# SchusterLab/qoc

Hardware: AMD Instinct MI355X
Metric: propagator-steps/sec (fwd+grad), dim=32 Schroedinger, 1000 steps x 256 seeds (higher is better)
Workload: dtype f64

## Files before the change

### qoc_amd/csrc/qocx_action.hip

```cpp
#include "qocx_action_core.h"

namespace qocx {

namespace action {

#define QOCX_SCALAR_MEM __attribute__((address_space(4)))
typedef const QOCX_SCALAR_MEM int* ScalarInts;
typedef const QOCX_SCALAR_MEM double* ScalarDoubles;

static __device__ __forceinline__ double inv_p(int p) {
    constexpr InvTable table;
    return table.v[p];
}

__device__ __forceinline__ void dpp_cmac16(double& r0, double& i0, double& r1, double& i1, double xr, double xi,
                                           const double (&ar)[16], const double (&ai)[16]) {
#define QOCX_ACTION_CMAC(R, I, C)                                                                          \
    "v_fmac_f64_dpp %[" R "], %[xr], %[ar" #C "] row_newbcast:" #C " row_mask:0xf bank_mask:0xf\n\t"         \
    "v_fmac_f64_dpp %[" I "], %[xi], %[ar" #C "] row_newbcast:" #C " row_mask:0xf bank_mask:0xf\n\t"         \
    "v_fmac_f64_dpp %[" R "], -%[xi], %[ai" #C "] row_newbcast:" #C " row_mask:0xf bank_mask:0xf\n\t"        \
    "v_fmac_f64_dpp %[" I "], %[xr], %[ai" #C "] row_newbcast:" #C " row_mask:0xf bank_mask:0xf\n\t"
#define QOCX_ACTION_CMAC2(C, D) QOCX_ACTION_CMAC("r0", "i0", C) QOCX_ACTION_CMAC("r1", "i1", D)
#define QOCX_ACTION_COL(C) [ar##C] "v"(ar[C]), [ai##C] "v"(ai[C])
    asm("s_nop 1\n\t" QOCX_ACTION_CMAC2(0, 1) QOCX_ACTION_CMAC2(2, 3) QOCX_ACTION_CMAC2(4, 5) QOCX_ACTION_CMAC2(6, 7)
            QOCX_ACTION_CMAC2(8, 9) QOCX_ACTION_CMAC2(10, 11) QOCX_ACTION_CMAC2(12, 13) QOCX_ACTION_CMAC2(14, 15)
        : [r0] "+v"(r0), [i0] "+v"(i0), [r1] "+v"(r1), [i1] "+v"(i1)
        : [xr] "v"(xr), [xi] "v"(xi), QOCX_ACTION_COL(0), QOCX_ACTION_COL(1), QOCX_ACTION_COL(2), QOCX_ACTION_COL(3),
          QOCX_ACTION_COL(4), QOCX_ACTION_COL(5), QOCX_ACTION_COL(6), QOCX_ACTION_COL(7), QOCX_ACTION_COL(8),
          QOCX_ACTION_COL(9), QOCX_ACTION_COL(10), QOCX_ACTION_COL(11), QOCX_ACTION_COL(12), QOCX_ACTION_COL(13),
          QOCX_ACTION_COL(14), QOCX_ACTION_COL(15));
#undef QOCX_ACTION_COL
#undef QOCX_ACTION_CMAC2
#undef QOCX_ACTION_CMAC
}

template <int NB, int KR, bool EXACT>
static __device__ __forceinline__ void action_sweep_body(const ActionArgs& args, double2* turn) {
    typedef Geo<NB> G;
    constexpr int NP = G::NP, CPL = G::CPL, H = G::H;
    const SweepArgs& sw = args.sw;
    const int b = blockIdx.x;
    const int lane = lane_id(), i = lane % NP, h = lane / NP;
    const bool g0 = (h == 0);
    const int nsteps = sw.nsteps, K = EXACT ? KR : args.K, m_max = args.m_max;
    const int jb = sw.j_begin, je = sw.j_end;
    const double dt = args.dt;
    __builtin_amdgcn_s_setprio(3);

    static_assert(NB == 2 && CPL == 16, "one block of 16 columns per lane group");
    auto image_at = [&](int cc) { return ((16 * h + cc) / H) * 64 + ((16 * h + cc) % H) * NP + i; };
    double h0r[CPL], h0i[CPL], gr[KR][CPL], gi[KR][CPL];
#pragma unroll
    for (int cc = 0; cc < CPL; ++cc) {
        const double2 e = args.h0_rimg[image_at(cc)];
        h0r[cc] = dt * e.y;
        h0i[cc] = -dt * e.x;
    }
#pragma unroll
    for (int k = 0; k < KR; ++k)
#pragma unroll
        for (int cc = 0; cc < CPL; ++cc) {
            const double2 e = k < K ? args.g_rimg[(size_t)k * G::MAT + image_at(cc)] : make_double2(0, 0);
            gr[k][cc] = dt * e.y;
            gi[k][cc] = -dt * e.x;
        }

    const ScalarInts words = (ScalarInts)(sw.s_arr + (size_t)b * nsteps);
    const ScalarDoubles u_b = (ScalarDoubles)(args.ustep + (size_t)b * nsteps * K);
    struct StepHead {
        int word;
        double u[KR];
    };
    auto fetch = [&](int step) __attribute__((always_inline)) {
        StepHead s;
        s.word = words[step];
#pragma unroll
        for (int k = 0; k < KR; ++k) s.u[k] = k < K ? u_b[(size_t)step * K + k] : 0.0;
        return s;
    };
    double are[CPL], aim[CPL];
    auto build = [&](int step, const StepHead& s) __attribute__((always_inline)) {
        if constexpr (EXACT) {
#pragma unroll
            for (int cc = 0; cc < CPL; ++cc) {
                double r = h0r[cc], im = h0i[cc];
#pragma unroll
                for (int k = 0; k < KR; ++k) {
                    r = fma(s.u[k], gr[k][cc], r);
                    im = fma(s.u[k], gi[k][cc], im);
                }
                are[cc] = r;
                aim[cc] = im;
            }
        } else {
#pragma unroll
            for (int cc = 0; cc < CPL; ++cc) {
                are[cc] = h0r[cc];
                aim[cc] = h0i[cc];
            }
#pragma unroll
            for (int k = 0; k < KR; ++k)
                if (k < K) {
                    const double uk = s.u[k];
#pragma unroll
                    for (int cc = 0; cc < CPL; ++cc) {
                        are[cc] = fma(uk, gr[k][cc], are[cc]);
                        aim[cc] = fma(uk, gi[k][cc], aim[cc]);
                    }
                }
            for (int k = KR; k < K; ++k) {
                const double uk = u_b[(size_t)step * K + k] * dt;
#pragma unroll
                for (int cc = 0; cc < CPL; ++cc) {
                    const double2 e = args.g_rimg[(size_t)k * G::MAT + image_at(cc)];
                    are[cc] = fma(uk, e.y, are[cc]);
                    aim[cc] = fma(-uk, e.x, aim[cc]);
                }
            }
        }
    };
    auto matvec = [&](double xr, double xi, double& yr, double& yi) __attribute__((always_inline)) {
        const double sxr = spread_halves(xr, h), sxi = spread_halves(xi, h);
        double s0r = 0, s0i = 0, s1r = 0, s1i = 0;
        dpp_cmac16(s0r, s0i, s1r, s1i, sxr, sxi, are, aim);
        yr = sum_groups<NB>(s0r + s1r);
        yi = sum_groups<NB>(s0i + s1i);
    };
    double vr = 0, vi = 0;
    int count = 0;
    auto step_apply = [&](int step, const StepHead& s, double sign, double2* keep_base)
                          __attribute__((always_inline)) {
        const int m = step_degree(__builtin_amdgcn_readfirstlane(s.word));
        if (m < 1 || m > m_max) return false;
        build(step, s);
        double2* keep = keep_base ? keep_base + ((size_t)b * nsteps + step) * m_max * NP : nullptr;
        count += (lane == m) ? 1 : 0;
        double sr = vr, si = vi;
        for (int p = 1; p <= m; ++p) {
            const double f = sign * inv_p(p);
            if (keep != nullptr && g0) keep[(size_t)(p - 1) * NP + i] = make_double2(vr, vi);
            double yr, yi;
            matvec(vr, vi, yr, yi);
            vr = f * yr;
            vi = f * yi;
            sr += vr;
            si += vi;
        }
        vr = sr;
        vi = si;
        return true;
    };
    auto refuse = [&]() {
        if (lane == 0) atomicOr(sw.status, 8);
    };

    if (sw.phase & 1) {
        const double2 p0 = jb == 0 ? sw.psi0[i] : args.carry_f[(size_t)b * NP + i];
        vr = p0.x;
        vi = p0.y;
        StepHead head = fetch(jb);
        for (int step = jb; step < je; ++step) {
            const StepHead next = fetch(step + 1 < je ? step + 1 : step);
            if (!step_apply(step, head, 1.0, args.kv_f)) {
                refuse();
                return;
            }
            head = next;
        }
        if (count > 0 && lane <= MMAX) atomicAdd(args.degree_counts + lane, count);
        if (je == nsteps) {
            turn[i] = make_double2(vr, vi);
            wave_sync();
            const double cost = eval_costs<NB>(sw, false, true, turn, nullptr, h, i);
            if (sw.unit_adjoint && sw.want_grad) unit_adjoint_scales<NB>(sw, turn, b, h, i);
            if (g0) sw.final_out[(size_t)b * NP + i] = make_double2(vr, vi);
            if (lane == 0) sw.cost_out[b] = cost;
        } else if (g0) {
            args.carry_f[(size_t)b * NP + i] = make_double2(vr, vi);
        }
    }
    if (!(sw.phase & 2)) return;

    wave_sync();
    if (je == nsteps) {
        unit_adjoint_seed<NB>(sw, turn, 0, 1, h, i);
        wave_sync();
        const double2 t = turn[i];
        vr = t.x;
        vi = t.y;
    } else {
        const double2 t = sw.lam_buf[(size_t)b * NP + i];
        vr = t.x;
        vi = t.y;
    }
    StepHead head = fetch(je - 1);
    for (int step = je - 1; step >= jb; --step) {
        const StepHead next = fetch(step - 1 >= jb ? step - 1 : step);
        if (!step_apply(step, head, -1.0, args.kv_b)) {
            refuse();
            return;
        }
        head = next;
    }
    if (jb > 0 && g0) sw.lam_buf[(size_t)b * NP + i] = make_double2(vr, vi);
}

template <int NB, int KR>
__global__ __launch_bounds__(64) void action_sweep_kernel(ActionArgs args) {
    __shared__ __attribute__((aligned(16))) double2 turn[Geo<NB>::NP];
    action_sweep_body<NB, KR, false>(args, turn);
}

template <int NB>
__global__ __launch_bounds__(64) void action_sweep_exact_kernel(ActionArgs args) {
    __shared__ __attribute__((aligned(16))) double2 turn[Geo<NB>::NP];
    action_sweep_body<NB, 2, true>(args, turn);
}

template <int NB>
__global__ __launch_bounds__(64) __attribute__((amdgpu_waves_per_eu(5, 5))) void action_grad_kernel(
    ActionGradArgs args) {
    typedef Geo<NB> G;
    constexpr int NP = G::NP, CPL = G::CPL, H = G::H, GB = 4;
    static_assert(H == 2, "the two lane groups share the terms of rho");
    extern __shared__ __attribute__((aligned(16))) char smem[];
    double2* vl = reinterpret_cast<double2*>(smem);
    double2* rho = vl + (size_t)args.m_max * NP;
    const int step = args.step0 + blockIdx.x, b = blockIdx.y;
    const int lane = lane_id(), i = lane % NP, h = lane / NP;
    const int K = args.K;
    const size_t idx = (size_t)b * args.nsteps + step;
    const int m = step_degree(args.s_arr[idx]);
    if (m < 1 || m > args.m_max) return;
    const double2* vf = args.kv_f + idx * args.m_max * NP;
    const double2* wb = args.kv_b + idx * args.m_max * NP;
    double2 tv = wb[i];
    for (int l0 = h; l0 < m + h; l0 += 4 * H) {
        double2 t[4];
#pragma unroll
        for (int q = 0; q < 4; ++q) t[q] = vf[(size_t)min(l0 + q * H, m - 1) * NP + i];
        asm volatile("" : "+v"(t[0].x), "+v"(t[0].y), "+v"(t[1].x), "+v"(t[1].y), "+v"(t[2].x), "+v"(t[2].y),
                          "+v"(t[3].x), "+v"(t[3].y));
#pragma unroll
        for (int q = 0; q < 4; ++q)
            if (l0 + q * H < m) vl[(l0 + q * H) * NP + i] = t[q];
    }
    double abr[CPL], abi[CPL];
#pragma unroll
    for (int cc = 0; cc < CPL; ++cc) {
        abr[cc] = 0;
        abi[cc] = 0;
    }
    wave_sync();
    for (int ii = 0; ii < m; ++ii) {
        double rr = 0, ri = 0;
        for (int l0 = 0; l0 < m - ii; l0 += H) {
            const double c0 = COEF.c[ii * MMAX + l0], c1 = COEF.c[ii * MMAX + l0 + 1];
            const double c = h == 0 ? c0 : c1;
            const int l = l0 + h;
            if (l < m - ii) {
                const double2 v = vl[l * NP + i];
                rr = fma(c, v.x, rr);
                ri = fma(c, v.y, ri);
            }
        }
        rr = sum_groups<NB>(rr);
        ri = sum_groups<NB>(ri);
        double2* slot = rho + (ii & 1) * NP;
        slot[i] = make_double2(rr, ri);
        wave_sync();
        const double2 w = tv;
        if (ii + 1 < m) tv = wb[(size_t)(ii + 1) * NP + i];
#pragma unroll
        for (int c0 = 0; c0 < CPL; c0 += GB) {
            double2 r[GB];
#pragma unroll
            for (int cc = 0; cc < GB; ++cc) r[cc] = slot[(c0 + cc) * H + h];
#pragma unroll
            for (int cc = 0; cc < GB; ++cc) {
                abr[c0 + cc] = fma(w.y, r[cc].y, fma(w.x, r[cc].x, abr[c0 + cc]));
                abi[c0 + cc] = fma(-w.x, r[cc].y, fma(w.y, r[cc].x, abi[c0 + cc]));
            }
        }
    }
    const double dts = args.dt;
    for (int k = 0; k < K; ++k) {
        double acc = 0, acc_im = 0;
#pragma unroll
        for (int c0 = 0; c0 < CPL; c0 += GB) {
            double2 e[GB];
#pragma unroll
            for (int cc = 0; cc < GB; ++cc) e[cc] = args.g_rimg[(size_t)k * G::MAT + (c0 + cc) * 64 + lane];
            asm volatile("" ::: "memory");
#pragma unroll
            for (int cc = 0; cc < GB; ++cc) {
                acc = fma(abi[c0 + cc], -dts * e[cc].x, fma(abr[c0 + cc], dts * e[cc].y, acc));
                acc_im = fma(abi[c0 + cc], -dts * e[cc].y, fma(abr[c0 + cc], -dts * e[cc].x, acc_im));
            }
        }
        acc = wave_sum(acc);
        acc_im = wave_sum(acc_im);
        if (lane == 0) {
            args.gstep[(idx * K + k) * 2] = acc;
            args.gstep[(idx * K + k) * 2 + 1] = acc_im;
        }
    }
}

}

int action_grad_lds_bytes(int m_max) { return (m_max + 2) * Geo<2>::NP * (int)sizeof(double2); }

void launch_action_sweep(const ActionArgs& a, int batch, hipStream_t st) {
    if (batch <= 0 || a.sw.j_end <= a.sw.j_begin) return;
    if (a.K == 2)
        hipLaunchKernelGGL((action::action_sweep_exact_kernel<2>), dim3(batch), dim3(64), 0, st, a);
    else
        hipLaunchKernelGGL((action::action_sweep_kernel<2, 2>), dim3(batch), dim3(64), 0, st, a);
}

void launch_action_grad(const ActionGradArgs& a, int nsteps, int batch, hipStream_t st) {
    if (batch <= 0 || nsteps <= 0) return;
    hipLaunchKernelGGL((action::action_grad_kernel<2>), dim3(nsteps, batch), dim3(64),
                       action_grad_lds_bytes(a.m_max), st, a);
}

}
```

### qoc_amd/csrc/qocx_action_core.h

```cpp
#ifndef QOCX_ACTION_CORE_H
#define QOCX_ACTION_CORE_H

#include "qocx_sweep_common.h"
#include "qocx_action.h"

namespace qocx {

namespace action {

constexpr int MMAX = QOCX_ACTION_MAX_DEGREE;

struct InvTable {
    double v[MMAX + 2];
    constexpr InvTable() : v{} {
        for (int p = 1; p < MMAX + 2; ++p) v[p] = 1.0 / (double)p;
    }
};
struct CoefTable {
    double c[MMAX * MMAX];
    constexpr CoefTable() : c{} {
        for (int i = 0; i < MMAX; ++i) {
            double v = 1.0 / (double)(i + 1);
            c[i * MMAX] = v;
            for (int l = 1; l < MMAX; ++l) {
                v = v * (double)l / (double)(i + l + 1);
                c[i * MMAX + l] = v;
            }
        }
    }
};
__device__ __constant__ const InvTable INV_P = InvTable();
__device__ __constant__ const CoefTable COEF = CoefTable();

template <int K0>
__device__ __forceinline__ void dpp_cmac4(double& r0, double& i0, double& r1, double& i1, double xr, double xi,
                                          double a0r, double a0i, double a1r, double a1i, double a2r,
                                          double a2i, double a3r, double a3i) {
#define QOCX_ACTION_CMAC(R, I, AR, AI, BC)                                                        \
    "v_fmac_f64_dpp %[" R "], %[xr], %[" AR "] row_newbcast:%[" BC "] row_mask:0xf bank_mask:0xf\n\t"  \
    "v_fmac_f64_dpp %[" I "], %[xi], %[" AR "] row_newbcast:%[" BC "] row_mask:0xf bank_mask:0xf\n\t"  \
    "v_fmac_f64_dpp %[" R "], -%[xi], %[" AI "] row_newbcast:%[" BC "] row_mask:0xf bank_mask:0xf\n\t" \
    "v_fmac_f64_dpp %[" I "], %[xr], %[" AI "] row_newbcast:%[" BC "] row_mask:0xf bank_mask:0xf\n\t"
    asm("s_nop 1\n\t" QOCX_ACTION_CMAC("r0", "i0", "a0r", "a0i", "k0") QOCX_ACTION_CMAC("r1", "i1", "a1r", "a1i", "k1")
            QOCX_ACTION_CMAC("r0", "i0", "a2r", "a2i", "k2") QOCX_ACTION_CMAC("r1", "i1", "a3r", "a3i", "k3")
        : [r0] "+v"(r0), [i0] "+v"(i0), [r1] "+v"(r1), [i1] "+v"(i1)
        : [xr] "v"(xr), [xi] "v"(xi), [a0r] "v"(a0r), [a0i] "v"(a0i), [a1r] "v"(a1r), [a1i] "v"(a1i),
          [a2r] "v"(a2r), [a2i] "v"(a2i), [a3r] "v"(a3r), [a3i] "v"(a3i), [k0] "i"(K0), [k1] "i"(K0 + 1),
          [k2] "i"(K0 + 2), [k3] "i"(K0 + 3));
#undef QOCX_ACTION_CMAC
}

__device__ __forceinline__ double spread_halves(double v, int h) {
    const unsigned lo = (unsigned)__double2loint(v), hi = (unsigned)__double2hiint(v);
    auto a = __builtin_amdgcn_permlane16_swap(lo, lo, false, false);
    auto b = __builtin_amdgcn_permlane16_swap(hi, hi, false, false);
    return h == 0 ? make_f64((int)a[0], (int)b[0]) : make_f64((int)a[1], (int)b[1]);
}

}

}

#endif
```

### qoc_amd/csrc/qocx_api.hip

```cpp
#include <dlfcn.h>
#include <unistd.h>

#include <cfloat>

#include "qocx_host.h"
#include "qocx_action.h"

namespace {

thread_local std::string g_error;

}

namespace qocx::host {

int fail(int code, const std::string& msg) {
    g_error = msg;
    return code;
}

const double THETA13 = 5.371920351148152;

int pade_scale_count(double norm1) {
    int s = 0;
// ... 1180 lines not shown
    }
    std::vector<double2> padded((size_t)batch * count * S * np, make_double2(0, 0));
    for (size_t v = 0; v < (size_t)batch * count * S; ++v)
        for (int i = 0; i < n; ++i)
            padded[v * np + i] = make_double2(bars[2 * (v * n + i)], bars[2 * (v * n + i) + 1]);
    if (ctx->inj_index.upload(index, ctx->stream) || ctx->inj_bars.upload(padded, ctx->stream))
        return QOCX_ERR_HIP;
    ctx->inj_count = count;
    ctx->inj_batch = batch;
    return 0;
}

int qocx_set_chunk(qocx_ctx* ctx, int32_t seeds_per_chunk) {
    if (!ctx) return fail(QOCX_ERR_ARG, "ctx is NULL");
    ctx->chunk_user = seeds_per_chunk < 0 ? 0 : seeds_per_chunk;
    return 0;
}

int qocx_set_pipeline(qocx_ctx* ctx, int32_t time_segments) {
    if (!ctx) return fail(QOCX_ERR_ARG, "ctx is NULL");
    ctx->pipe_user = time_segments < 0 ? 0 : time_segments;
    return 0;
}

int qocx_set_keep_step_states(qocx_ctx* ctx, int32_t keep) {
    if (!ctx) return fail(QOCX_ERR_ARG, "ctx is NULL");
    ctx->keep_step_states = keep ? 1 : 0;
    return 0;
}

static int eval_seeds(qocx_ctx* ctx, int32_t want_grad) {
    if (ctx->seeds.M == 0) return eval_items(ctx, want_grad);
    if (!ctx->has_problem || ctx->B < 1) return fail(QOCX_ERR_STATE, "no problem / controls");
    HIP_TRY(hipSetDevice(ctx->device));
    const int seeds = ctx->ens_B;
    if (ctx->ens_stale)
        if (int rc = ensemble_expand(ctx, seeds)) return rc;
    if (int rc = eval_items(ctx, want_grad)) return rc;
    if (ctx->ens_cost.ensure((size_t)seeds) ||
        (ctx->have_grads && ctx->ens_grads.ensure((size_t)seeds * ctx->nc * ctx->seeds.Kr)))
        return QOCX_ERR_HIP;
    SeedBuffers buf = seed_buffers(ctx);
    if (!ctx->have_grads) buf.grads = nullptr;
    if (ctx->seeds.sweep()) qocx::launch_sweep_reduce(sweep_args(ctx->seeds, ctx->nc, buf), ctx->stream);
    else qocx::launch_ensemble_reduce(ensemble_args(ctx->seeds, seeds, ctx->nc, buf), ctx->stream);
    HIP_TRY(hipGetLastError());
    HIP_TRY(hipStreamSynchronize(ctx->stream));
    return 0;
}

int qocx_eval_resident(qocx_ctx* ctx, int32_t want_grad) {
    if (!ctx) return fail(QOCX_ERR_ARG, "ctx is NULL");
    if (int rc = eval_seeds(ctx, want_grad)) return rc;
    ControlCosts& cc = ctx->control_costs;
    if (cc.count == 0) return duration_finish(ctx);
    const int seeds = seed_count(ctx);
    if (int rc = run_control_costs(ctx, cc, seeds, ctx->nc, seed_channels(ctx), seed_controls(ctx), ctx->have_grads))
        return rc;
    qocx::launch_add_control_costs(seed_costs(ctx), cc.cost.p, ctx->have_grads ? seed_grads(ctx) : nullptr,
                                   cc.grad.p, seeds, (size_t)ctx->nc * seed_channels(ctx), ctx->stream);
    HIP_TRY(hipGetLastError());
    HIP_TRY(hipStreamSynchronize(ctx->stream));
    return duration_finish(ctx);
}

int qocx_download_results(qocx_ctx* ctx, double* cost_out, double* grad_out, double* final_out) {
    if (!ctx) return fail(QOCX_ERR_ARG, "ctx is NULL");
    if (!ctx->have_results) return fail(QOCX_ERR_STATE, "no evaluation results");
    HIP_TRY(hipSetDevice(ctx->device));
    const int B = ctx->B, np = ctx->np, S = ctx->S, n = ctx->n, seeds = seed_count(ctx);
    if (cost_out)
        HIP_TRY(hipMemcpyAsync(cost_out, seed_costs(ctx), (size_t)seeds * sizeof(double),
                               hipMemcpyDeviceToHost, ctx->stream));
    if (grad_out) {
        if (!ctx->have_grads) return fail(QOCX_ERR_STATE, "gradients were not computed");
        HIP_TRY(hipMemcpyAsync(grad_out, seed_grads(ctx),
                               (size_t)seeds * ctx->nc * seed_channels(ctx) * sizeof(double),
                               hipMemcpyDeviceToHost, ctx->stream));
    }
    std::vector<double2> fin;
    if (final_out) {
        fin.resize((size_t)B * S * np);
        HIP_TRY(hipMemcpyAsync(fin.data(), ctx->final_out.p, fin.size() * sizeof(double2),
                               hipMemcpyDeviceToHost, ctx->stream));
    }
    HIP_TRY(hipStreamSynchronize(ctx->stream));
    if (final_out)
        for (size_t v = 0; v < (size_t)B * S; ++v)
            for (int i = 0; i < n; ++i) {
                final_out[2 * (v * n + i)] = fin[v * np + i].x;
                final_out[2 * (v * n + i) + 1] = fin[v * np + i].y;
            }
    return 0;
}

int qocx_download_step_states(qocx_ctx* ctx, double* states_out) {
    if (!ctx || !states_out) return fail(QOCX_ERR_ARG, "NULL argument");
    if (!ctx->have_results || !ctx->have_step_states)
        return fail(QOCX_ERR_STATE, "step states were not kept (qocx_set_keep_step_states)");
    HIP_TRY(hipSetDevice(ctx->device));
    const size_t nvec = (size_t)ctx->B * (ctx->nsteps + 1) * ctx->S;
    std::vector<double2> tmp(nvec * ctx->np);
    HIP_TRY(hipMemcpy(tmp.data(), ctx->step_states.p, tmp.size() * sizeof(double2),
                      hipMemcpyDeviceToHost));
    for (size_t v = 0; v < nvec; ++v)
        for (int i = 0; i < ctx->n; ++i) {
            states_out[2 * (v * ctx->n + i)] = tmp[v * ctx->np + i].x;
            states_out[2 * (v * ctx->n + i) + 1] = tmp[v * ctx->np + i].y;
        }
    return 0;
}

int qocx_eval_schroedinger(qocx_ctx* ctx, int32_t batch, const double* controls, int32_t want_grad,
                           double* cost_out, double* grad_out, double* final_out) {
    int rc = qocx_upload_controls(ctx, batch, controls);
    if (rc) return rc;
    rc = eval_seeds(ctx, want_grad);
    if (rc) return rc;
    if ((rc = duration_finish(ctx))) return rc;
    return qocx_download_results(ctx, cost_out, (want_grad && ctx->K > 0) ? grad_out : nullptr,
                                 final_out);
}

int qocx_set_timing(qocx_ctx* ctx, int32_t enable) {
    if (!ctx) return fail(QOCX_ERR_ARG, "ctx is NULL");
    if (enable < 0 || enable > 8) return fail(QOCX_ERR_ARG, "timing mode must be 0, 1 or 2 + kernel index");
    ctx->timing = enable;
    ctx->time_active = false;
    return 0;
}

int qocx_get_timing(qocx_ctx* ctx, int32_t which, int64_t* launches, double* total_ms) {
    if (!ctx || which < 0 || which > 6) return fail(QOCX_ERR_ARG, "bad argument");
    if (launches) *launches = ctx->t_launch[which];
    if (total_ms) *total_ms = ctx->t_ms[which];
    return 0;
}

int qocx_reset_timing(qocx_ctx* ctx) {
    if (!ctx) return fail(QOCX_ERR_ARG, "ctx is NULL");
    for (int i = 0; i < 7; ++i) {
        ctx->t_launch[i] = 0;
        ctx->t_ms[i] = 0;
    }
    return 0;
}

static const char* const kVariantKnobs[] = {
    "sweep_impl", "sweep_one", "sweep_dense", "sweep_inverse", "sweep_inverse_small", "sweep_umode", "bidir",
    "unit_adjoint", "latency", "fuse_lu", "lu_inverse", "lu_mfma", "lu_dpp", "pack8", "m4_linear", "magnus_4w",
    "pade_order", "k1a_three", "k1a_four", "k1a_share", "k1a_herm4", "general_split", "general_skew",
    "lindblad_two_sided", "lindblad_side_limit", "lindblad_q2", "lindblad_chain", "lindblad_real_ops", "lindblad_4t",
    "lindblad_hermitian", "lindblad_pad_operator", "action", "action_states", "action_costs",
    "action_degree"};
static const char* const kDiagKnobs[] = {"dbg_skip", "sweep3_dbg", "sweep3_stamps", "lindblad_stamps",
                                         "k1a_stamps", "k1a_dbg", "peak_mode"};

int qocx_knob_kind(const char* name) {
    if (!name) return 0;
    for (const char* k : kVariantKnobs)
        if (strcmp(k, name) == 0) return 1;
    for (const char* k : kDiagKnobs)
        if (strcmp(k, name) == 0) return qocx::kDiagBuild ? 2 : -2;
    return 0;
}

int qocx_build_is_diag(void) { return qocx::kDiagBuild ? 1 : 0; }

int qocx_debug_set_knob(qocx_ctx* ctx, const char* name, int64_t value) {
    if (!ctx || !name) return fail(QOCX_ERR_ARG, "NULL argument");
    const int kind = qocx_knob_kind(name);
    if (kind > 0) {
        if (strcmp(name, "action_states") == 0 && value != 0 && (value < 2 || value > QOCX_ACTION_MAX_STATES))
            return fail(QOCX_ERR_ARG, "action_states must be 0 or 2 .. 4 (QOCX_ACTION_MAX_STATES)");
        if (strcmp(name, "action_costs") == 0 && value != 0 && value != 1)
            return fail(QOCX_ERR_ARG, "action_costs must be 0 or 1");
        if (strcmp(name, "action_degree") == 0 && value != 0 && value != 1)
            return fail(QOCX_ERR_ARG, "action_degree must be 0 or 1");
        ctx->knobs[name] = value;
        return 0;
    }
    if (kind == -2)
        return fail(QOCX_ERR_ARG, std::string("diagnostic knob '") + name +
                                      "' exists in libqocx_diag.so only (make diag, -DQOCX_DIAG)");
    return fail(QOCX_ERR_ARG, std::string("unknown knob: ") + name);
}


int qocx_comm_unique_id(uint8_t* id128) {
    if (!id128) return fail(QOCX_ERR_ARG, "id128 is NULL");
    qocx_ctx tmp;
    int rc = load_rccl(&tmp);
    if (rc) return rc;
    int e = tmp.rccl.GetUniqueId((void*)id128);
    if (e != 0) return fail(QOCX_ERR_RCCL, "ncclGetUniqueId failed");
    return 0;
}

int qocx_comm_init(qocx_ctx* ctx, const uint8_t* id128, int32_t rank, int32_t world) {
    if (!ctx || !id128) return fail(QOCX_ERR_ARG, "NULL argument");
    HIP_TRY(hipSetDevice(ctx->device));
    int rc = load_rccl(ctx);
    if (rc) return rc;
    typedef int (*init_fn)(void**, int, ncclUniqueIdBytes, int);
    init_fn f = (init_fn)dlsym(ctx->rccl.lib, "ncclCommInitRank");
    ncclUniqueIdBytes uid;
    memcpy(uid.internal, id128, 128);
    if (world < 1 || rank < 0 || rank >= world) return fail(QOCX_ERR_ARG, "rank / world out of range");
    if (!f) return fail(QOCX_ERR_RCCL, "librccl has no ncclCommInitRank");
    if (getenv("QOCX_RCCL_DEBUG")) {
        unsigned long long sum = 1469598103934665603ull;
        for (int i = 0; i < 128; ++i) sum = (sum ^ id128[i]) * 1099511628211ull;
        char bus[64] = "?";
        (void)hipDeviceGetPCIBusId(bus, sizeof(bus), ctx->device);
        int version = 0;
        typedef int (*ver_fn)(int*);
        if (ver_fn v = (ver_fn)dlsym(ctx->rccl.lib, "ncclGetVersion")) (void)v(&version);
        const char* ipc = getenv("HSA_ENABLE_IPC_MODE_LEGACY");
        fprintf(stderr, "[qocx rccl] ncclCommInitRank rank=%d world=%d hip_device=%d pci=%s id_fnv=%016llx "
                        "rccl_version=%d HSA_ENABLE_IPC_MODE_LEGACY=%s pid=%d\n",
                rank, world, ctx->device, bus, sum, version, ipc ? ipc : "(unset)", (int)getpid());
        fflush(stderr);
    }
    int e = f(&ctx->comm, world, uid, rank);
    if (e != 0)
        return fail(QOCX_ERR_RCCL, std::string("ncclCommInitRank: ") +
                                       (ctx->rccl.GetErrorString ? ctx->rccl.GetErrorString(e) : "?"));
    return 0;
}

static int comm_allreduce(qocx_ctx* ctx, double* buf, int64_t count, int op) {
    if (!ctx || !buf || count < 1) return fail(QOCX_ERR_ARG, "bad argument");
    if (!ctx->comm) return fail(QOCX_ERR_STATE, "communicator not initialised");
    HIP_TRY(hipSetDevice(ctx->device));
    if (ctx->comm_buf.ensure((size_t)count)) return QOCX_ERR_HIP;
    HIP_TRY(hipMemcpyAsync(ctx->comm_buf.p, buf, count * sizeof(double), hipMemcpyHostToDevice,
                           ctx->stream));
    int e = ctx->rccl.AllReduce(ctx->comm_buf.p, ctx->comm_buf.p, (size_t)count, 8, op, ctx->comm,
                                ctx->stream);
    if (e != 0)
        return fail(QOCX_ERR_RCCL, std::string("ncclAllReduce: ") +
                                       (ctx->rccl.GetErrorString ? ctx->rccl.GetErrorString(e) : "?"));
    HIP_TRY(hipMemcpyAsync(buf, ctx->comm_buf.p, count * sizeof(double), hipMemcpyDeviceToHost,
                           ctx->stream));
    HIP_TRY(hipStreamSynchronize(ctx->stream));
    return 0;
}

int qocx_download_costs(qocx_ctx* ctx, double* cost_out) {
    if (!ctx || !cost_out) return fail(QOCX_ERR_ARG, "NULL argument");
    if (!ctx->have_results) return fail(QOCX_ERR_STATE, "no evaluation results");
    HIP_TRY(hipSetDevice(ctx->device));
    HIP_TRY(hipMemcpyAsync(cost_out, seed_costs(ctx), (size_t)seed_count(ctx) * sizeof(double),
                           hipMemcpyDeviceToHost, ctx->stream));
    HIP_TRY(hipStreamSynchronize(ctx->stream));
    return 0;
}

int qocx_ensemble_download_members(qocx_ctx* ctx, double* cost_out) {
    if (!ctx || !cost_out) return fail(QOCX_ERR_ARG, "NULL argument");
    if (ctx->seeds.M == 0 || ctx->seeds.swp_B > 0) return fail(QOCX_ERR_STATE, "no ensemble set (qocx_set_ensemble)");
    if (!ctx->have_results) return fail(QOCX_ERR_STATE, "no evaluation results");
    HIP_TRY(hipSetDevice(ctx->device));
    HIP_TRY(hipMemcpyAsync(cost_out, ctx->cost_out.p, (size_t)ctx->B * sizeof(double),
                           hipMemcpyDeviceToHost, ctx->stream));
    HIP_TRY(hipStreamSynchronize(ctx->stream));
    return 0;
}

int qocx_sweep_download_sensitivities(qocx_ctx* ctx, double* scales_out, double* offsets_out) {
    if (!ctx) return fail(QOCX_ERR_ARG, "ctx is NULL");
    if (ctx->seeds.swp_B == 0) return fail(QOCX_ERR_STATE, "no sweep set (qocx_set_sweep)");
    if (!ctx->have_results || !ctx->have_grads || ctx->ens_stale)
        return fail(QOCX_ERR_STATE, "sweep sensitivities need an evaluation with gradients");
    HIP_TRY(hipSetDevice(ctx->device));
    const size_t ns = (size_t)ctx->seeds.swp_B * ctx->seeds.Kr, no = (size_t)ctx->seeds.swp_B * ctx->seeds.J;
    if (ctx->seeds.scale_sens.ensure(ns) || ctx->seeds.offset_sens.ensure(no)) return QOCX_ERR_HIP;
    qocx::launch_sweep_sensitivity(sweep_args(ctx), ctx->stream);
    HIP_TRY(hipGetLastError());
    if (scales_out)
        HIP_TRY(hipMemcpyAsync(scales_out, ctx->seeds.scale_sens.p, ns * sizeof(double), hipMemcpyDeviceToHost,
                               ctx->stream));
    if (offsets_out && no > 0)
        HIP_TRY(hipMemcpyAsync(offsets_out, ctx->seeds.offset_sens.p, no * sizeof(double), hipMemcpyDeviceToHost,
                               ctx->stream));
    HIP_TRY(hipStreamSynchronize(ctx->stream));
    return 0;
}

int qocx_sweep_set_durations(qocx_ctx* ctx, const double* tau, const double* base_scales,
                             const double* base_offsets, double tau_min, double tau_max, double time_weight) {
    if (!ctx || !tau) return fail(QOCX_ERR_ARG, "NULL argument");
    if (!ctx->seeds.sweep()) return fail(QOCX_ERR_STATE, "no sweep set (qocx_set_sweep before qocx_sweep_set_durations)");
    HIP_TRY(hipSetDevice(ctx->device));
    std::vector<double> s0, d0;
    if (int rc = set_seed_durations(ctx->seeds, tau, base_scales, base_offsets, tau_min, tau_max, time_weight,
                                    ctx->stream, s0, d0))
        return rc;
    qocx::launch_duration_tables(duration_args(ctx->seeds, nullptr, nullptr), ctx->stream);
    HIP_TRY(hipGetLastError());
    if (int rc = sweep_mirror_tables(ctx)) return rc;
    seed_tables_were_set(ctx, s0, d0, tau_max);
    ctx->seeds.dur.set = true;
    ctx->seeds.dur.have_grad = false;
    return 0;
}

int qocx_sweep_download_durations(qocx_ctx* ctx, double* tau_out, double* tau_grad_out) {
    if (!ctx) return fail(QOCX_ERR_ARG, "ctx is NULL");
    if (!ctx->seeds.dur.set) return fail(QOCX_ERR_STATE, "no durations set (qocx_sweep_set_durations)");
    HIP_TRY(hipSetDevice(ctx->device));
    const bool stands = ctx->have_results && ctx->have_grads && !ctx->ens_stale && ctx->seeds.dur.have_grad;
    return download_seed_durations(ctx->seeds, ctx->stream, stands, tau_out, tau_grad_out);
}

int qocx_reduce_results(qocx_ctx* ctx, int32_t allreduce, double* out, int64_t count) {
    if (!ctx || !out) return fail(QOCX_ERR_ARG, "NULL argument");
    if (!ctx->have_results) return fail(QOCX_ERR_STATE, "no evaluation results");
    if (allreduce && !ctx->comm) return fail(QOCX_ERR_STATE, "communicator not initialised");
    const int per_seed = count > 1 ? ctx->nc * seed_channels(ctx) : 0;
    if (count != 1 + per_seed || (per_seed > 0 && !ctx->have_grads))
        return fail(QOCX_ERR_ARG, "count must be 1, or 1 + control_eval_count * control_count after "
                                  "an evaluation with gradients");
    HIP_TRY(hipSetDevice(ctx->device));
    if (ctx->comm_buf.ensure((size_t)count)) return QOCX_ERR_HIP;
    qocx::launch_reduce_results(seed_costs(ctx), seed_grads(ctx), seed_count(ctx), per_seed, ctx->comm_buf.p,
                                ctx->stream);
    if (allreduce) {
        int e = ctx->rccl.AllReduce(ctx->comm_buf.p, ctx->comm_buf.p, (size_t)count, 8, 0, ctx->comm,
                                    ctx->stream);
        if (e != 0)
// ... 31 lines not shown
```

### qoc_amd/csrc/qocx_host_resident.hip

```cpp
#include "qocx_host.h"
#include "qocx_action.h"

namespace qocx {
size_t general_krylov_scratch(int np, int S);
void launch_general_magnus(const MagnusArgs& a, bool vjp, int blocks, hipStream_t st);
}
static constexpr int kActionRefused = -0x7a11;
static int finish_items(qocx_ctx* ctx, int want_grad) {
    HIP_TRY(hipGetLastError());
    int status = 0;
    HIP_TRY(hipMemcpyAsync(&status, ctx->status.p, sizeof(int), hipMemcpyDeviceToHost, ctx->stream));
    HIP_TRY(hipStreamSynchronize(ctx->stream));
    time_collect(ctx);
    if (status & 8) return kActionRefused;
    if (status & 2) return fail(QOCX_ERR_ARG, "non-finite generator norm");
    if (status & 1) return fail(QOCX_ERR_SINGULAR, "Singular matrix");
    if (status & 4) return fail(QOCX_ERR_CAPACITY, "squaring sub-step capacity exceeded");
    ctx->have_results = true;
    ctx->have_grads = want_grad != 0;
    ctx->have_step_states = ctx->keep_step_states != 0;
    return 0;
}

using EffKind = EffectiveControls::Kind;
// ... 544 lines not shown
        if (r.action) {
            aa.ustep = ctx->ustep.p; aa.h0_rimg = ctx->h0.r.p; aa.g_rimg = ctx->g.r.p;
            aa.K = ctx->K; aa.m_max = r.m_max; aa.dt = ctx->dt;
            aa.kv_f = want_grad ? ctx->kry_f.p : nullptr;
            aa.kv_b = want_grad ? ctx->kry_b.p : nullptr;
            aa.carry_f = ctx->action_carry.p;
            aa.degree_counts = ctx->action_counts.p;
            ga.kv_f = ctx->kry_f.p; ga.kv_b = ctx->kry_b.p; ga.s_arr = ctx->s_arr.p; ga.g_rimg = ctx->g.r.p;
            ga.K = ctx->K; ga.m_max = r.m_max; ga.nsteps = nsteps; ga.dt = ctx->dt; ga.gstep = ctx->gstep.p;
            sga.S = S;
        }
        return 0;
    }

    int factor_segment(int i) {
        const int nb = ctx->nb, np = ctx->np, plo = lo[i], len = lo[i + 1] - lo[i];
        if (r.action) {
            if (nseg > 1) HIP_TRY(hipEventRecord(ctx->ev_factored[i], cs));
            return 0;
        }
        fa.step0 = plo; fa.seg_len = len;
        time_begin(ctx, 0, cs);
        if (ctx->explicit_mode) {
            qocx::launch_pq_explicit(nb, ctx->gen_rm.p + (size_t)b0 * ctx->nsteps * np * np, np, fa,
                                     bc * len, cs);
        } else if (r.nodes > 1) {
            ma.step0 = plo; ma.seg_len = len; ma.total = (size_t)bc * len;
            ma.m_rm = ctx->m_rm.p; ma.mbar_rm = nullptr; ma.gstep = nullptr;
            if (r.magnus4w) qocx::launch_magnus4w_fwd(ma, bc, cs);
            else qocx::launch_magnus_fwd(nb, ma, (int)std::min<size_t>(ma.total, 1024), cs);
            qocx::launch_pq_explicit(nb, ma.m_rm, np, fa, bc * len, cs);
        } else {
            qocx::launch_pq(nb, fa, len, bc, cs);
        }
        time_end(ctx, cs);
        if (!ctx->explicit_mode && r.nodes == 1 && qocx::pq_second_pending(nb, fa, len)) {
            HIP_TRY(hipEventRecord(ctx->ev_pq[i], cs));
            HIP_TRY(hipStreamWaitEvent(ctx->lu_stream, ctx->ev_pq[i], 0));
            time_begin(ctx, 4, ctx->lu_stream);
            qocx::launch_pq3_second(fa, len, bc, ctx->lu_stream);
            time_end(ctx, ctx->lu_stream);
            HIP_TRY(hipEventRecord(ctx->ev_factored[i], ctx->lu_stream));
            if (nseg <= 1) HIP_TRY(hipStreamWaitEvent(cs, ctx->ev_factored[i], 0));
            return 0;
        }
        la.step0 = plo; la.seg_len = len;
        if (!r.fused_lu && nb == 4 && nseg > 1 && ctx->lu_stream != nullptr) {
            HIP_TRY(hipEventRecord(ctx->ev_pq[i], cs));
            HIP_TRY(hipStreamWaitEvent(ctx->lu_stream, ctx->ev_pq[i], 0));
            time_begin(ctx, 4, ctx->lu_stream);
            qocx::launch_lu(nb, la, (size_t)bc * len, ctx->lu_stream);
            time_end(ctx, ctx->lu_stream);
            HIP_TRY(hipEventRecord(ctx->ev_factored[i], ctx->lu_stream));
            return 0;
        }
        if (!r.fused_lu) {
            time_begin(ctx, 4, cs);
            qocx::launch_lu(nb, la, la.pack8 ? (size_t)bc * ((len + 1) / 2) : (size_t)bc * len, cs);
            if (r.umode) qocx::launch_umul(nb, la, fa.q_img, ctx->qt_img.p, (size_t)bc * len, cs);
            time_end(ctx, cs);
        }
        if (nseg > 1) HIP_TRY(hipEventRecord(ctx->ev_factored[i], cs));
        return 0;
    }

    void sweep(int jb, int je, int phase, hipStream_t st) {
        sa.j_begin = jb; sa.j_end = je; sa.phase = phase;
        time_begin(ctx, 1, st);
        if (!((dbg_skip & 1) && (phase & 1)) && !((dbg_skip & 2) && (phase & 2))) {
            if (r.action) {
                aa.sw = sa;
                if (r.action_costs) qocx::launch_action_costs_sweep(aa, bc, st);
                else if (ctx->S > 1) qocx::launch_action_states_sweep(aa, bc, st);
                else if (ctx->nb == 2) qocx::launch_action_sweep(aa, bc, st);
                else qocx::launch_action4_sweep(ctx->n, aa, bc, st);
            } else if (r.dense) qocx::launch_sweepd(sa, bc, st);
            else if (r.inverse_sweep) qocx::launch_sweepi(ctx->nb, sa, bc, st);
            else if (r.sweep3) qocx::launch_sweep3(ctx->nb, sa, bc, st);
            else qocx::launch_sweep(ctx->nb, sa, bc, st);
        }
        time_end(ctx, st);
    }

    void krylov(int jb, int je) {
        const int len = je - jb;
        ka.step0 = jb;
        time_begin(ctx, 2, cs);
        if (r.action) {
            ga.step0 = jb;
            if (dbg_skip & 4) {
            } else if (r.action_costs) {
                qocx::launch_action_costs_grad(ga, len, bc, cs);
            } else if (ctx->S > 1) {
                sga.g = ga;
                qocx::launch_action_states_grad(sga, len, bc, cs);
            } else if (ctx->nb == 2) qocx::launch_action_grad(ga, len, bc, cs);
            else qocx::launch_action4_grad(ctx->n, ga, len, bc, cs);
        } else if (!(dbg_skip & 4)) qocx::launch_krylov(ctx->nb, ka, len, bc, cs);
        if (r.nodes > 1) {
            ma.step0 = jb; ma.seg_len = len; ma.total = (size_t)bc * len;
            ma.m_rm = nullptr; ma.mbar_rm = ka.mbar_rm; ma.gstep = ka.gstep;
            if (r.magnus4w) qocx::launch_magnus4w_vjp(ma, bc, cs);
            else qocx::launch_magnus_vjp(ctx->nb, ma, (int)std::min<size_t>(ma.total, 1024), cs);
        }
        time_end(ctx, cs);
    }
};

int run_one_sided(ResidentChunk& c) {
    qocx_ctx* ctx = c.ctx;
    const int nseg = c.nseg;
    for (int i = 0; i < nseg; ++i) {
        if (int rc = c.factor_segment(i)) return rc;
        if (nseg > 1) HIP_TRY(hipStreamWaitEvent(c.ss, ctx->ev_factored[i], 0));
        c.sweep(c.lo[i], c.lo[i + 1], (nseg == 1 && c.want_grad) ? 3 : 1, c.ss);
    }
    if (nseg > 1 && c.want_grad) {
        for (int i = nseg - 1; i >= 0; --i) {
            c.sweep(c.lo[i], c.lo[i + 1], 2, c.ss);
            HIP_TRY(hipEventRecord(ctx->ev_swept[i], c.ss));
        }
    } else if (nseg > 1) {
        HIP_TRY(hipEventRecord(ctx->ev_swept[0], c.ss));
        HIP_TRY(hipStreamWaitEvent(c.cs, ctx->ev_swept[0], 0));
    }
    if (c.want_grad)
        for (int i = nseg - 1; i >= 0; --i) {
            if (nseg > 1) HIP_TRY(hipStreamWaitEvent(c.cs, ctx->ev_swept[i], 0));
            c.krylov(c.lo[i], c.lo[i + 1]);
        }
    return 0;
}

int run_two_sided(ResidentChunk& c) {
    qocx_ctx* ctx = c.ctx;
    const int nseg = c.nseg;
    const std::vector<int>& lo = c.lo;
    hipStream_t sf = ctx->sweep_streams[0], sb = ctx->sweep_streams[1];
    const bool small_launch = (size_t)c.bc * ctx->nsteps < 16384;
    int parts_out = small_launch ? 1 : 3;
    if ((nseg - 2) + 2 * parts_out > (int)ctx->ev_fwd.size()) parts_out = 1;
    struct Piece { int lo, hi; };
    std::vector<Piece> piece;
    std::vector<int> first(nseg + 1, 0);
    for (int i = 0; i < nseg; ++i) {
        const int np_i = (i == 0 || i == nseg - 1) ? parts_out : 1;
        first[i] = (int)piece.size();
        for (int part = 0; part < np_i; ++part)
            piece.push_back({lo[i] + (int)((int64_t)(lo[i + 1] - lo[i]) * part / np_i),
                             lo[i] + (int)((int64_t)(lo[i + 1] - lo[i]) * (part + 1) / np_i)});
    }
    first[nseg] = (int)piece.size();
    const int P = (int)piece.size();
    std::vector<char> factored(nseg, 0);
    int next_f = 0, next_b = nseg - 1;
    const bool adj_first = small_launch;
    for (int t = 0; t < nseg; ++t) {
        const bool back = adj_first ? (t % 2 == 0) : (t % 2 == 1);
        const int i = back ? nseg - 1 - t / 2 : t / 2;
        if (int rc = c.factor_segment(i)) return rc;
        factored[i] = 1;
        while (next_f < nseg && factored[next_f]) {
            HIP_TRY(hipStreamWaitEvent(sf, ctx->ev_factored[next_f], 0));
            for (int p = first[next_f]; p < first[next_f + 1]; ++p) {
                if (piece[p].hi > piece[p].lo) c.sweep(piece[p].lo, piece[p].hi, 1, sf);
                HIP_TRY(hipEventRecord(ctx->ev_fwd[p], sf));
            }
            ++next_f;
        }
        while (next_b >= 0 && factored[next_b]) {
            HIP_TRY(hipStreamWaitEvent(sb, ctx->ev_factored[next_b], 0));
            for (int p = first[next_b + 1] - 1; p >= first[next_b]; --p) {
                if (piece[p].hi > piece[p].lo) c.sweep(piece[p].lo, piece[p].hi, 2, sb);
                HIP_TRY(hipEventRecord(ctx->ev_swept[p], sb));
            }
            --next_b;
        }
    }
    const int mid = first[nseg / 2];
    for (int d = 0; d < P; ++d)
        for (int p : {mid + d, mid - 1 - d}) {
            if (p < 0 || p >= P || piece[p].hi <= piece[p].lo) continue;
            HIP_TRY(hipStreamWaitEvent(c.cs, ctx->ev_fwd[p], 0));
            HIP_TRY(hipStreamWaitEvent(c.cs, ctx->ev_swept[p], 0));
            c.krylov(piece[p].lo, piece[p].hi);
        }
    return 0;
}

}

namespace qocx::host {

static int eval_resident(qocx_ctx* ctx, int32_t want_grad, bool allow_action);

int eval_items(qocx_ctx* ctx, int32_t want_grad) {
    if (!ctx->has_problem || ctx->B < 1) return fail(QOCX_ERR_STATE, "no problem / controls");
    HIP_TRY(hipSetDevice(ctx->device));
    const int B = ctx->B;
    const bool explicit_gen = ctx->explicit_mode;
    want_grad = (want_grad && (ctx->K > 0 || explicit_gen)) ? 1 : 0;
    if (explicit_gen && want_grad)
        if (ctx->genbar_rm.ensure((size_t)B * ctx->nsteps * ctx->np * ctx->np)) return QOCX_ERR_HIP;
    if (ctx->inj_count > 0 && ctx->inj_batch != B)
        return fail(QOCX_ERR_STATE, "state cotangents were set for a different batch size");
    if (ctx->action_counts.p != nullptr)
        HIP_TRY(hipMemsetAsync(ctx->action_counts.p, 0, ctx->action_counts.count * sizeof(int), ctx->stream));
    if (ctx->general_path) return eval_general(ctx, want_grad);
    int rc = eval_resident(ctx, want_grad, true);
    if (rc == kActionRefused) {
        ctx->action_reruns += 1;
        rc = eval_resident(ctx, want_grad, false);
    }
    return rc;
}

int eval_resident(qocx_ctx* ctx, int32_t want_grad, bool allow_action) {
    const int B = ctx->B;
    const ResidentRoute route = resident_route(ctx, want_grad, allow_action);
    int chunk = 0;
    if (int rc = reserve_resident(ctx, route, want_grad, chunk)) return rc;
    HIP_TRY(hipMemsetAsync(ctx->status.p, 0, sizeof(int), ctx->stream));
    HIP_TRY(hipMemsetAsync(ctx->action_counts.p, 0, ctx->action_counts.count * sizeof(int), ctx->stream));
    for (int b0 = 0; b0 < B; b0 += chunk) {
        ResidentChunk c(ctx, route, want_grad, b0, std::min(chunk, B - b0));
        ctx->last_chunk = c.bc;
        if (int rc = c.init()) return rc;
        if (int rc = c.two_sided ? run_two_sided(c) : run_one_sided(c)) return rc;
        if (want_grad) scatter_gradients(ctx, c.eff, c.ka.gstep, c.lam_scale(), b0, c.bc, c.cs);
    }
    return finish_items(ctx, want_grad);
}

}
```

Measured before the change: 85.28 million.

## Spread state across lane halves with permlane reductions and fuse inward action sweeps

The action kernel now gives each lane a spread state index, so the matvec no longer needs the spread_halves broadcast before the DPP multiply-accumulates. It then reduces partial sums with permlane16/permlane32 swaps in place of the group sum. On the host, a new default-on action_plan knob issues one forward sweep launch covering every piece before the midpoint, and one backward launch covering every piece after it, instead of one launch per piece. This cuts launch and event overhead and lets each sweep run longer. The trade-off is that the fused launches wait only on the first (or last) segment's factored event, and indexing now relies on the new lane-to-state mapping.

```diff
diff --git a/qoc_amd/csrc/qocx_action.hip b/qoc_amd/csrc/qocx_action.hip
--- a/qoc_amd/csrc/qocx_action.hip
+++ b/qoc_amd/csrc/qocx_action.hip
@@ -41,7 +41,8 @@
     const SweepArgs& sw = args.sw;
     const int b = blockIdx.x;
     const int lane = lane_id(), i = lane % NP, h = lane / NP;
-    const bool g0 = (h == 0);
+    const int idx = spread_index(lane);
+    const bool holder = spread_holder(lane);
     const int nsteps = sw.nsteps, K = EXACT ? KR : args.K, m_max = args.m_max;
     const int jb = sw.j_begin, je = sw.j_end;
     const double dt = args.dt;
@@ -120,11 +121,9 @@
         }
     };
     auto matvec = [&](double xr, double xi, double& yr, double& yi) __attribute__((always_inline)) {
-        const double sxr = spread_halves(xr, h), sxi = spread_halves(xi, h);
         double s0r = 0, s0i = 0, s1r = 0, s1i = 0;
-        dpp_cmac16(s0r, s0i, s1r, s1i, sxr, sxi, are, aim);
-        yr = sum_groups<NB>(s0r + s1r);
-        yi = sum_groups<NB>(s0i + s1i);
+        dpp_cmac16(s0r, s0i, s1r, s1i, xr, xi, are, aim);
+        sum_spread2(s0r + s1r, s0i + s1i, yr, yi);
     };
     double vr = 0, vi = 0;
     int count = 0;
@@ -138,7 +137,7 @@
         double sr = vr, si = vi;
         for (int p = 1; p <= m; ++p) {
             const double f = sign * inv_p(p);
-            if (keep != nullptr && g0) keep[(size_t)(p - 1) * NP + i] = make_double2(vr, vi);
+            if (keep != nullptr && holder) keep[(size_t)(p - 1) * NP + idx] = make_double2(vr, vi);
             double yr, yi;
             matvec(vr, vi, yr, yi);
             vr = f * yr;
@@ -155,7 +154,7 @@
     };
 
     if (sw.phase & 1) {
-        const double2 p0 = jb == 0 ? sw.psi0[i] : args.carry_f[(size_t)b * NP + i];
+        const double2 p0 = jb == 0 ? sw.psi0[idx] : args.carry_f[(size_t)b * NP + idx];
         vr = p0.x;
         vi = p0.y;
         StepHead head = fetch(jb);
@@ -169,14 +168,14 @@
         }
         if (count > 0 && lane <= MMAX) atomicAdd(args.degree_counts + lane, count);
         if (je == nsteps) {
-            turn[i] = make_double2(vr, vi);
+            turn[idx] = make_double2(vr, vi);
             wave_sync();
             const double cost = eval_costs<NB>(sw, false, true, turn, nullptr, h, i);
             if (sw.unit_adjoint && sw.want_grad) unit_adjoint_scales<NB>(sw, turn, b, h, i);
-            if (g0) sw.final_out[(size_t)b * NP + i] = make_double2(vr, vi);
+            if (holder) sw.final_out[(size_t)b * NP + idx] = make_double2(vr, vi);
             if (lane == 0) sw.cost_out[b] = cost;
-        } else if (g0) {
-            args.carry_f[(size_t)b * NP + i] = make_double2(vr, vi);
+        } else if (holder) {
+            args.carry_f[(size_t)b * NP + idx] = make_double2(vr, vi);
         }
     }
     if (!(sw.phase & 2)) return;
@@ -185,11 +184,11 @@
     if (je == nsteps) {
         unit_adjoint_seed<NB>(sw, turn, 0, 1, h, i);
         wave_sync();
-        const double2 t = turn[i];
+        const double2 t = turn[idx];
         vr = t.x;
         vi = t.y;
     } else {
-        const double2 t = sw.lam_buf[(size_t)b * NP + i];
+        const double2 t = sw.lam_buf[(size_t)b * NP + idx];
         vr = t.x;
         vi = t.y;
     }
@@ -202,7 +201,7 @@
         }
         head = next;
     }
-    if (jb > 0 && g0) sw.lam_buf[(size_t)b * NP + i] = make_double2(vr, vi);
+    if (jb > 0 && holder) sw.lam_buf[(size_t)b * NP + idx] = make_double2(vr, vi);
 }
 
 template <int NB, int KR>
diff --git a/qoc_amd/csrc/qocx_action_core.h b/qoc_amd/csrc/qocx_action_core.h
--- a/qoc_amd/csrc/qocx_action_core.h
+++ b/qoc_amd/csrc/qocx_action_core.h
@@ -57,6 +57,24 @@
     return h == 0 ? make_f64((int)a[0], (int)b[0]) : make_f64((int)a[1], (int)b[1]);
 }
 
+__device__ __forceinline__ int spread_index(int lane) { return 16 * (lane >> 5) + (lane & 15); }
+__device__ __forceinline__ bool spread_holder(int lane) { return (lane & 16) == 0; }
+
+__device__ __forceinline__ void sum_spread2(double pr, double pi, double& yr, double& yi) {
+    const unsigned rl = (unsigned)__double2loint(pr), rh = (unsigned)__double2hiint(pr);
+    const unsigned il = (unsigned)__double2loint(pi), ih = (unsigned)__double2hiint(pi);
+    auto a = __builtin_amdgcn_permlane16_swap(rl, rl, false, false);
+    auto b = __builtin_amdgcn_permlane16_swap(rh, rh, false, false);
+    auto c = __builtin_amdgcn_permlane16_swap(il, il, false, false);
+    auto d = __builtin_amdgcn_permlane16_swap(ih, ih, false, false);
+    auto e = __builtin_amdgcn_permlane32_swap(a[0], a[1], false, false);
+    auto f = __builtin_amdgcn_permlane32_swap(b[0], b[1], false, false);
+    auto g = __builtin_amdgcn_permlane32_swap(c[0], c[1], false, false);
+    auto k = __builtin_amdgcn_permlane32_swap(d[0], d[1], false, false);
+    yr = make_f64((int)e[0], (int)f[0]) + make_f64((int)e[1], (int)f[1]);
+    yi = make_f64((int)g[0], (int)k[0]) + make_f64((int)g[1], (int)k[1]);
+}
+
 }
 
 }
diff --git a/qoc_amd/csrc/qocx_api.hip b/qoc_amd/csrc/qocx_api.hip
--- a/qoc_amd/csrc/qocx_api.hip
+++ b/qoc_amd/csrc/qocx_api.hip
@@ -1356,7 +1356,7 @@
     "pade_order", "k1a_three", "k1a_four", "k1a_share", "k1a_herm4", "general_split", "general_skew",
     "lindblad_two_sided", "lindblad_side_limit", "lindblad_q2", "lindblad_chain", "lindblad_real_ops", "lindblad_4t",
     "lindblad_hermitian", "lindblad_pad_operator", "action", "action_states", "action_costs",
-    "action_degree"};
+    "action_degree", "action_plan"};
 static const char* const kDiagKnobs[] = {"dbg_skip", "sweep3_dbg", "sweep3_stamps", "lindblad_stamps",
                                          "k1a_stamps", "k1a_dbg", "peak_mode"};
 
@@ -1381,6 +1381,8 @@
             return fail(QOCX_ERR_ARG, "action_costs must be 0 or 1");
         if (strcmp(name, "action_degree") == 0 && value != 0 && value != 1)
             return fail(QOCX_ERR_ARG, "action_degree must be 0 or 1");
+        if (strcmp(name, "action_plan") == 0 && value != 0 && value != 1)
+            return fail(QOCX_ERR_ARG, "action_plan must be 0 or 1");
         ctx->knobs[name] = value;
         return 0;
     }
diff --git a/qoc_amd/csrc/qocx_host_resident.hip b/qoc_amd/csrc/qocx_host_resident.hip
--- a/qoc_amd/csrc/qocx_host_resident.hip
+++ b/qoc_amd/csrc/qocx_host_resident.hip
@@ -720,6 +720,8 @@
     }
     first[nseg] = (int)piece.size();
     const int P = (int)piece.size();
+    const int mid = first[nseg / 2];
+    const bool fuse_inward = c.r.action && ctx->knob("action_plan", 1) != 0;
     std::vector<char> factored(nseg, 0);
     int next_f = 0, next_b = nseg - 1;
     const bool adj_first = small_launch;
@@ -730,6 +732,12 @@
         factored[i] = 1;
         while (next_f < nseg && factored[next_f]) {
             HIP_TRY(hipStreamWaitEvent(sf, ctx->ev_factored[next_f], 0));
+            if (fuse_inward && next_f == 0) {
+                if (piece[mid - 1].hi > piece[0].lo) c.sweep(piece[0].lo, piece[mid - 1].hi, 1, sf);
+                for (int p = 0; p < mid; ++p) HIP_TRY(hipEventRecord(ctx->ev_fwd[p], sf));
+                next_f = nseg / 2;
+                continue;
+            }
             for (int p = first[next_f]; p < first[next_f + 1]; ++p) {
                 if (piece[p].hi > piece[p].lo) c.sweep(piece[p].lo, piece[p].hi, 1, sf);
                 HIP_TRY(hipEventRecord(ctx->ev_fwd[p], sf));
@@ -738,6 +746,12 @@
         }
         while (next_b >= 0 && factored[next_b]) {
             HIP_TRY(hipStreamWaitEvent(sb, ctx->ev_factored[next_b], 0));
+            if (fuse_inward && next_b == nseg - 1) {
+                if (piece[P - 1].hi > piece[mid].lo) c.sweep(piece[mid].lo, piece[P - 1].hi, 2, sb);
+                for (int p = P - 1; p >= mid; --p) HIP_TRY(hipEventRecord(ctx->ev_swept[p], sb));
+                next_b = nseg / 2 - 1;
+                continue;
+            }
             for (int p = first[next_b + 1] - 1; p >= first[next_b]; --p) {
                 if (piece[p].hi > piece[p].lo) c.sweep(piece[p].lo, piece[p].hi, 2, sb);
                 HIP_TRY(hipEventRecord(ctx->ev_swept[p], sb));
@@ -745,7 +759,6 @@
             --next_b;
         }
     }
-    const int mid = first[nseg / 2];
     for (int d = 0; d < P; ++d)
         for (int p : {mid + d, mid - 1 - d}) {
             if (p < 0 || p >= P || piece[p].hi <= piece[p].lo) continue;
```

New measurement: 88.95 million (median of 6 runs). 4.3% higher.
